# JuliaDSP/DSP.jl

Measured on NVIDIA H100. Metric: Gsamples/s filt+welch on 2^26 cplx-F32, higher is better.
Workload: dtype c64 (ComplexF32; f32 arithmetic)

## Files before the change

### __graft_entry__.py

```python
import os
import subprocess
import sys

ROOT = os.path.dirname(os.path.abspath(__file__))
PKG = os.path.join(ROOT, "dsp.jl_b200")


def build() -> None:
    jobs = str(min(8, os.cpu_count() or 2))
    subprocess.run(["make", "-C", os.path.join(PKG, "csrc"), "-j", jobs], check=True)
    host_dir = os.path.join(ROOT, "tests", "host")
    os.makedirs(os.path.join(ROOT, "build"), exist_ok=True)
    subprocess.run(["g++", "-std=c++17", "-O2", "-x", "c++", "-w", "-I/usr/local/cuda/include",
                    "-o", os.path.join(ROOT, "build", "fft_core_host_check"),
                    os.path.join(host_dir, "fft_core_host_check.cu")], check=True)
    for name in ("fir_tile_host_check", "fir_state_host_check"):
        subprocess.run(["g++", "-std=c++17", "-O2", "-march=native", "-x", "c++", "-w", "-I/usr/local/cuda/include",
                        "-o", os.path.join(ROOT, "build", name), os.path.join(host_dir, name + ".cu")], check=True)
    if ROOT not in sys.path:
        sys.path.insert(0, ROOT)
    import dspb200
    assert dspb200._lib.lib.dspb200_version() == 100


def smoke() -> None:
    if ROOT not in sys.path:
        sys.path.insert(0, ROOT)
    import numpy as np
    import dspb200
    from oracle import dspbase as od, periodograms as op, windows as ow

    if dspb200.device_count() < 1:
        raise RuntimeError("smoke() needs a CUDA device; dspb200 has no CPU fallback")
    rng = np.random.default_rng(7)
    x = (rng.standard_normal(1 << 16) + 1j * rng.standard_normal(1 << 16)).astype(np.complex64)
    v = (rng.standard_normal(513) + 1j * rng.standard_normal(513)).astype(np.complex64)
    y = dspb200.conv(x, v, algorithm="fft_overlapsave")
    ref = od.conv_exact(x, v)
    err = np.linalg.norm(y - ref) / np.linalg.norm(ref)
    assert y.dtype == np.complex64 and err < 1e-6, f"conv parity {err}"
    s = rng.standard_normal(1 << 18).astype(np.float32)
    p = dspb200.welch_pgram(s, 4096, 2048, window=dspb200.hanning)
    pref, _ = op.welch_pgram(s, 4096, 2048, window=ow.hanning, f64=True)
    err2 = np.linalg.norm(p.power - pref) / np.linalg.norm(pref)
    assert p.power.dtype == np.float32 and err2 < 1e-6, f"welch parity {err2}"
    print(f"smoke ok: conv relerr {err:.2e}, welch relerr {err2:.2e}, launches {dspb200.launch_count()}")


# ... 5 lines not shown
```

### dsp.jl_b200/csrc/fft_core.cuh

```cuda
#pragma once
#include "common.cuh"
#include <math.h>

#ifndef DSP_PROBE
#define DSP_PROBE 0
#endif

namespace dspb200 {

template <typename T> struct fft_pad { static constexpr int K = sizeof(T) == 4 ? 2 : 1; };
template <typename T> __host__ __device__ constexpr int fft_pad256(int n) {
    if (sizeof(T) == 4) return n == 512 ? 8 : (n == 1024 ? 4 : (n == 8192 ? 4 : 2));
    return n == 512 ? 4 : (n == 1024 ? 2 : (n == 8192 ? 2 : 1));
}
template <typename T> __host__ __device__ constexpr int fft_pad4096(int n) {
    if (sizeof(T) == 4) return n == 8192 ? 2 : (n == 16384 ? 4 : 0);
    return n == 8192 ? 1 : 0;
}
template <typename T, int N> __host__ __device__ __forceinline__ constexpr int padaddr(int p) {
    return p + fft_pad<T>::K * (p >> 4) + fft_pad256<T>(N) * (p >> 8) + fft_pad4096<T>(N) * (p >> 12);
}
template <typename T> __host__ __device__ constexpr int padded_len(int n) {
    return ((n - 1) + fft_pad<T>::K * ((n - 1) >> 4) + fft_pad256<T>(n) * ((n - 1) >> 8) + fft_pad4096<T>(n) * ((n - 1) >> 12) + 1 + 3) & ~3;
}
// ... 441 lines not shown
    } else {
        const int t = tp + Q * A;
        cx<T> w[RL / 2];
        if constexpr (N == 16384) {
            const cx<T> w1 = fft_tl_in_smem<T, N>() ? c.tl[t] : ldtw<T>(c.tl, t);
            w[1] = w1;
            w[0] = mkc<T>(fma_(w1.x, w1.x, -(w1.y * w1.y)), (w1.x + w1.x) * w1.y);
        } else {
#pragma unroll
            for (int i = 0; i < P::TLK; ++i) w[i] = fft_tl_in_smem<T, N>() ? c.tl[t * P::TLK + i] : ldtw<T>(c.tl, t * P::TLK + i);
        }
        fft_bfly<T, RL, false>(u, w);
    }
}

template <typename T, int N, int NT, class Ld0, class StLast>
__device__ __forceinline__ void fft_forward(const FftCtx<T>& c, int tid, Ld0 ld0, StLast stlast) {
    constexpr int Q = fft_plan_traits<N>::Q;
    constexpr int ITERS = (Q + NT - 1) / NT;
    fft_first_pass<T, N, NT, false>(c, tid, ld0);
    __syncthreads();
    fft_middle<T, N, NT>(c, tid);
#pragma unroll
    for (int it = 0; it < ITERS; ++it) {
        const int tp = tid + it * NT;
        if (Q % NT != 0 && tp >= Q) break;
        cx<T> v[16];
        fft_last_pass<T, N>(c, tp, v);
#pragma unroll
        for (int r = 0; r < 16; ++r) stlast(tp + r * Q, it, r, v[r]);
    }
}

template <typename T> inline void fft_fill_row(cx<T>* row, int R, long long num, long long den, int limit = 1 << 30) {
    const long double PI2 = 6.283185307179586476925286766559005768L;
    int qb = 0;
    for (int r = R; r > 1; r >>= 1) ++qb;
    int idx = 0;
    for (int k = 1; k <= qb; ++k) {
        const int cnt = k <= 2 ? 1 : (1 << (k - 2));
        for (int m = 0; m < cnt; ++m) {
            const long double a = -PI2 * ((long double)num * (long double)(R >> k) / (long double)den + (long double)m / (long double)(1 << k));
            if (idx < limit) row[idx] = mkc<T>((T)cosl(a), (T)sinl(a));
            ++idx;
        }
    }
}
template <typename T> inline void fft_fill_tables(cx<T>* t16, cx<T>* t256, long long n) {
    cx<T> row[8];
    const int nrow = fft_tw_row(n);
    const int keep6[6] = {0, 1, 2, 4, 5, 7};
    for (int t = 0; t < 16; ++t) {
        fft_fill_row<T>(row, 16, t, 256);
        for (int i = 0; i < nrow; ++i) t16[fft_tw_index<T>(i, t, 16)] = row[nrow == 8 ? i : keep6[i]];
    }
    for (int t = 0; t < 256; ++t) {
        fft_fill_row<T>(row, 16, t, 4096);
        for (int i = 0; i < nrow; ++i) t256[fft_tw_index<T>(i, t, 256)] = row[nrow == 8 ? i : keep6[i]];
    }
}
inline void fft_last_radix(long long n, int* rl, int* tlk) {
    int logn = 0;
    for (long long m = n; m > 1; m >>= 1) ++logn;
    const int ql = logn - 4;
    const int nmid = ql <= 4 ? 0 : (ql <= 8 ? 1 : 2);
    *rl = 1 << (ql - 4 * nmid);
    *tlk = *rl == 16 ? 0 : (n == 16384 ? 1 : *rl / 2);
}
inline long long fft_tl_len_rt(long long n) {
    int rl, tlk;
    fft_last_radix(n, &rl, &tlk);
    return (n / rl) * tlk;
}
template <typename T> inline void fft_fill_tl(cx<T>* tl, long long n) {
    int rl, tlk;
    fft_last_radix(n, &rl, &tlk);
    if (tlk == 0) return;
    const long double PI2 = 6.283185307179586476925286766559005768L;
    for (long long t = 0; t < n / rl; ++t) {
        if (n == 16384) {
            const long double a = -PI2 * (long double)t / (long double)n;
            tl[t] = mkc<T>((T)cosl(a), (T)sinl(a));
        } else {
            fft_fill_row<T>(tl + t * tlk, rl, t, n);
        }
    }
}

template <int N> struct fft_threads {
    static constexpr int NB16 = N / 16;
    static constexpr int value = NB16 < 64 ? 64 : (NB16 > 512 ? 512 : (NB16 > 256 ? 256 : NB16));
};
template <typename T, int N> struct fft_minblocks {
    static constexpr int value = sizeof(T) == 8 ? 1 : (fft_threads<N>::value >= 512 ? 1 : 512 / fft_threads<N>::value);
};

}
```

### dsp.jl_b200/csrc/overlap_save.cu

```cuda
#include "fft_core.cuh"
#include "async_copy.cuh"
#include "cufft_exec.cuh"
#include <math.h>
#include <stdlib.h>
#include <new>

namespace dspb200 {

struct OsPlanImpl {
    int dtype = 0;
    bool cplx = false, f64 = false;
    int64_t nv = 0, nfft = 0, L = 0;
    bool fused = false;
    int device = 0;
    void* d_tw = nullptr;
    void* d_t16 = nullptr;
    void* d_t256 = nullptr;
    int sm_count = 0;
    int fused_per_sm = 0;
    int fused_state_per_sm = 0;
    void* d_H = nullptr;
    cufftHandle fwd = 0, inv = 0;
    bool fft_ok = false;
    int64_t batch = 0, nbins = 0;
    DevBuf td, fd;
    HostPipe pipe;
};

template <typename T, bool CPLX> struct os_elt { using type = T; };
template <typename T> struct os_elt<T, true> { using type = cx<T>; };


template <typename T, int N, bool CPLX> struct os_threads {
    static constexpr bool f32 = sizeof(T) == 4;
    static constexpr int value = fft_threads<N>::value;
    static constexpr bool wide = f32 && ((N >= 512 && N <= 4096) || (N == 256 && !CPLX));
    static constexpr int minblocks = wide ? 1024 / value : fft_minblocks<T, N>::value;
    static constexpr bool staged = f32 && N == 16384;
};
constexpr int OS_STAGE_HEAD = 32768;
static_assert(OS_STAGE_HEAD % 16 == 0, "TMA copies move multiples of 16 bytes");
static_assert(OS_STAGE_HEAD < 16384 * 4, "the head region holds less than the shortest staged span (N + 1 floats)");
template <typename T, int N, bool CPLX> constexpr size_t os_smem_bytes() {
    return (size_t)fft_smem_elems<T, N>() * sizeof(cx<T>) + (os_threads<T, N, CPLX>::staged ? OS_STAGE_HEAD + 16 : 0);
}

template <typename T> __device__ __forceinline__ cx<T> ldg_cx(const cx<T>* __restrict__ p) {
    if constexpr (sizeof(T) == 4) {
        const float2 v = __ldg(reinterpret_cast<const float2*>(p));
        return mkc<T>(v.x, v.y);
    } else {
        const double2 v = __ldg(reinterpret_cast<const double2*>(p));
        return mkc<T>(v.x, v.y);
    }
}

template <typename E> struct OsUnit {
    const E* u;
    E* out;
    int jlo, jhi, jend, jzero;
    int nvm1, L;
};

template <typename E, bool STATE> struct OsState {};
template <typename E> struct OsState<E, true> {
    const E* si_in;
    E* si_out;
    int64_t nx;
};
template <typename E> struct OsUnitState {
    const E* si_in;
    E* si_out;
    int jsi, jnx;
};
struct OsNoState {};
template <typename E> __device__ __forceinline__ void os_put_state(const OsUnit<E>& g, const OsUnitState<E>& s, int j, E v) {
    if (j < s.jsi) v = v + s.si_in[j];
// ... 2 lines not shown
}

__device__ __forceinline__ int os_clamp(int64_t v) {
    return (int)(v < -(int64_t(1) << 30) ? -(int64_t(1) << 30) : (v > (int64_t(1) << 30) ? (int64_t(1) << 30) : v));
}
__device__ __forceinline__ int os_clamp_diff(int64_t a, int64_t b) {
    return a >= (int64_t(1) << 62) ? (1 << 30) : os_clamp(a - b);
}

template <typename T, bool CPLX, bool INTERIOR>
__device__ __forceinline__ cx<T> os_sample(const OsUnit<typename os_elt<T, CPLX>::type>& g, int j) {
#if DSP_PROBE & 2
    return mkc<T>(T(j), T(1));
#endif
    if constexpr (CPLX) {
        if constexpr (INTERIOR) return g.u[j];
        return (j >= g.jlo && j < g.jhi) ? g.u[j] : mkc<T>(T(0), T(0));
    } else {
        const int jb = j + g.L;
        if constexpr (INTERIOR) return mkc<T>(g.u[j], g.u[jb]);
        const T a = (j >= g.jlo && j < g.jhi) ? g.u[j] : T(0);
        const T b = (jb >= g.jlo && jb < g.jhi) ? g.u[jb] : T(0);
        return mkc<T>(a, b);
    }
}

struct OsStage {
    unsigned char* head;
    uint64_t* bar;
    uint32_t bytes;
    uint32_t parity;
};

template <typename T, int N, bool CPLX, int NT, bool INTERIOR, int ITERS, bool STATE, typename SG>
__device__ __forceinline__ void os_unit(const FftCtx<T>& ctx, int tid, const OsUnit<typename os_elt<T, CPLX>::type>& g,
                                        const cx<T>* __restrict__ H, OsStage& st, bool staged,
                                        const typename os_elt<T, CPLX>::type* __restrict__ next_u, const SG& state_geometry) {
    using E = typename os_elt<T, CPLX>::type;
    constexpr int Q = fft_plan_traits<N>::Q;
    constexpr bool STAGED = os_threads<T, N, CPLX>::staged;
    static_assert(ITERS == (Q + NT - 1) / NT, "register tile does not match the thread count");
    static_assert(!STAGED || (ITERS == 2 && Q % NT == 0), "TMA staging is laid out for two butterflies per thread");
    if (STAGED && INTERIOR && staged) {
        mbar_wait(st.bar, st.parity);
        st.parity ^= 1;
        const E* s = reinterpret_cast<const E*>(st.head);
        cx<T> v[ITERS][16];
#pragma unroll
        for (int it = 0; it < ITERS; ++it)
#pragma unroll
            for (int r = 0; r < 16; ++r) {
                const int j = tid + it * NT + r * Q;
                if constexpr (CPLX) v[it][r] = s[j];
                else v[it][r] = mkc<T>(s[j], s[j + g.L]);
            }
        fft_first_pass_regs<T, N, NT, true>(ctx, tid, v);
    } else {
        auto ld0 = [&](int j, int, int) -> cx<T> { return os_sample<T, CPLX, INTERIOR>(g, j); };
        fft_first_pass<T, N, NT, true>(ctx, tid, ld0);
    }
    __syncthreads();
    if (STAGED && next_u != nullptr && tid == 0) {
        fence_proxy_async_shared();
        mbar_expect_tx_noarrive(st.bar, OS_STAGE_HEAD);
        tma_load_1d(st.head, next_u, OS_STAGE_HEAD, st.bar);
    }
    fft_middle<T, N, NT>(ctx, tid);
    cx<T> v[ITERS][16];
#pragma unroll
    for (int it = 0; it < ITERS; ++it) {
        const int tp = tid + it * NT;
        if (Q % NT == 0 || tp < Q) {
            fft_last_pass<T, N, (ITERS == 1 && Q % NT == 0) ? NT : 0>(ctx, tp, v[it], tid);
#pragma unroll
#if DSP_PROBE & 4
            for (int r = 0; r < 16; ++r) v[it][r] = cswap(cmul(v[it][r], mkc<T>(T(0.5), T(r))));
#else
            for (int r = 0; r < 16; ++r) v[it][r] = cswap(cmul(v[it][r], ldg_cx<T>(H + tp + r * Q)));
#endif
            fft_bfly16_plain<T>(v[it]);
        }
    }
    __syncthreads();
#pragma unroll
    for (int it = 0; it < ITERS; ++it) {
        const int tp = tid + it * NT;
        if (Q % NT == 0 || tp < Q) fft_store_block<T, N>(ctx.sm, tp, v[it]);
    }
    __syncthreads();
    fft_middle<T, N, NT>(ctx, tid);
    constexpr int RL = fft_plan_traits<N>::RL, NBF = 16 / RL;
    using SGeom = std::conditional_t<STATE && !INTERIOR, OsUnitState<E>, OsNoState>;
    SGeom sg{};
    if constexpr (STATE && !INTERIOR) sg = state_geometry();
    auto put = [&](int j, cx<T> y) {
#if DSP_PROBE & 8
        if (y.x != T(123456.75)) return;
#endif
        if (j < g.nvm1) return;
        if constexpr (CPLX) {
            if constexpr (INTERIOR) g.out[j] = mkc<T>(y.y, y.x);
            else if constexpr (STATE) { if (j < g.jend) os_put_state(g, sg, j, mkc<T>(y.y, y.x)); }
            else if (j < g.jend) g.out[j] = (j < g.jzero) ? mkc<T>(y.y, y.x) : mkc<T>(T(0), T(0));
        } else {
            const int jb = j + g.L;
            if constexpr (INTERIOR) {
                g.out[j] = y.y;
                g.out[jb] = y.x;
            } else if constexpr (STATE) {
                if (j < g.jend) os_put_state(g, sg, j, y.y);
                if (jb < g.jend) os_put_state(g, sg, jb, y.x);
            } else {
                if (j < g.jend) g.out[j] = (j < g.jzero) ? y.y : T(0);
                if (jb < g.jend) g.out[jb] = (jb < g.jzero) ? y.x : T(0);
            }
        }
    };
    if constexpr (STAGED) {
        cx<T> w[ITERS][16];
#pragma unroll
        for (int it = 0; it < ITERS; ++it) fft_last_pass_load<T, N>(ctx, tid + it * NT, w[it]);
        if (next_u != nullptr) {
            __syncthreads();
            if (tid == 0) {
                fence_proxy_async_shared();
                mbar_expect_tx(st.bar, st.bytes - OS_STAGE_HEAD);
                tma_load_1d(ctx.sm, reinterpret_cast<const unsigned char*>(next_u) + OS_STAGE_HEAD, st.bytes - OS_STAGE_HEAD,
                            st.bar);
            }
        }
#pragma unroll
        for (int it = 0; it < ITERS; ++it) {
            const int tp = tid + it * NT;
            fft_last_pass_bfly<T, N>(ctx, tp, w[it]);
#pragma unroll
            for (int r = 0; r < 16; ++r) put(tp + r * Q, w[it][r]);
        }
    } else {
        auto chunk = [&](auto a_, int tp) {
            constexpr int A = decltype(a_)::value;
            cx<T> u[RL];
            fft_last_pass_chunk<T, N, A>(ctx, tp, u);
#pragma unroll
            for (int jj = 0; jj < RL; ++jj) put(tp + (A + NBF * jj) * Q, u[jj]);
        };
#pragma unroll
        for (int it = 0; it < ITERS; ++it) {
            const int tp = tid + it * NT;
            if (Q % NT != 0 && tp >= Q) break;
            chunk(std::integral_constant<int, 0>{}, tp);
            if constexpr (NBF >= 2) chunk(std::integral_constant<int, 1>{}, tp);
            if constexpr (NBF >= 4) { chunk(std::integral_constant<int, 2>{}, tp); chunk(std::integral_constant<int, 3>{}, tp); }
            if constexpr (NBF >= 8) {
                chunk(std::integral_constant<int, 4>{}, tp); chunk(std::integral_constant<int, 5>{}, tp);
                chunk(std::integral_constant<int, 6>{}, tp); chunk(std::integral_constant<int, 7>{}, tp);
            }
        }
    }
}

template <typename T, int N, bool CPLX, bool STATE>
__global__ void __launch_bounds__((os_threads<T, N, CPLX>::value), (os_threads<T, N, CPLX>::minblocks))
os_fused_kernel(const void* __restrict__ u_, int64_t u_begin, int64_t nu_local, int64_t u_col_stride,
                void* __restrict__ out_, int64_t out_begin, int64_t out_count, int64_t out_col_stride,
                int64_t zero_from, int nv, int64_t units_per_col, int64_t total_units, const cx<T>* __restrict__ gtl,
                const cx<T>* __restrict__ g16, const cx<T>* __restrict__ g256, const cx<T>* __restrict__ H,
                const OsState<typename os_elt<T, CPLX>::type, STATE> sa) {
    constexpr int NT = os_threads<T, N, CPLX>::value;
    constexpr int Q = fft_plan_traits<N>::Q;
    constexpr int ITERS = (Q + NT - 1) / NT;
    constexpr bool STAGED = os_threads<T, N, CPLX>::staged;
    extern __shared__ __align__(16) unsigned char smem_raw[];
    constexpr int HEAD = STAGED ? OS_STAGE_HEAD : 0;
    cx<T>* sm = reinterpret_cast<cx<T>*>(smem_raw + HEAD);
    using E = typename os_elt<T, CPLX>::type;
    const int tid = threadIdx.x;
    pdl_launch_dependents();
    const FftCtx<T> ctx = fft_make_ctx<T, N, NT>(sm, g16, g256, gtl, tid);
    OsStage st;
    st.head = smem_raw;
    st.bar = reinterpret_cast<uint64_t*>(smem_raw + HEAD + (size_t)fft_smem_elems<T, N>() * sizeof(cx<T>));
    st.parity = 0;
    if constexpr (STAGED) {
        if (tid == 0) {
            mbar_init(st.bar, 1);
            mbar_fence_init();
        }
    }
    pdl_wait();
    __syncthreads();
    const int L = N - nv + 1;
    const int span = CPLX ? N : N + L;
    st.bytes = (uint32_t)((span * sizeof(E) + 15) & ~(size_t)15);

    const bool onecol = units_per_col >= total_units;
    auto geometry = [&](int64_t gu, OsUnit<E>& g) -> bool {
        const int64_t col = onecol ? 0 : gu / units_per_col;
        const int64_t unit = gu - col * units_per_col;
        const int64_t q = CPLX ? unit : 2 * unit;
        const int64_t s0 = out_begin + q * L - (nv - 1);
        const int64_t i0 = s0 - u_begin;
        g.u = reinterpret_cast<const E*>(u_) + col * u_col_stride + i0;
        g.out = reinterpret_cast<E*>(out_) + col * out_col_stride + (s0 - out_begin);
        g.jlo = os_clamp(-i0);
        g.jhi = os_clamp(nu_local - i0);
        g.jend = os_clamp(out_begin + out_count - s0);
        g.jzero = os_clamp_diff(zero_from, s0);
        g.nvm1 = nv - 1;
        g.L = L;
        return g.jlo <= 0 && g.jhi >= span && g.jend >= span && g.jzero >= span;
    };
    auto state_geometry = [&](int64_t gu) {
        OsUnitState<E> s{};
        if constexpr (STATE) {
// ... 14 lines not shown
            int64_t lo = out_begin + qn * L - (nv - 1) - u_begin;
            int64_t hi = lo + span;
            if (lo < 0) lo = 0;
            if (hi > nu_local) hi = nu_local;
            const uintptr_t a0 = ((uintptr_t)(reinterpret_cast<const E*>(u_) + coln * u_col_stride + lo) + 15) & ~(uintptr_t)15;
            const uintptr_t a1 = (uintptr_t)(reinterpret_cast<const E*>(u_) + coln * u_col_stride + hi) & ~(uintptr_t)15;
            if (hi > lo && a1 > a0) tma_prefetch_l2(reinterpret_cast<const void*>(a0), (uint32_t)(a1 - a0));
        }
    };
    auto stage_src = [&](int64_t gn) -> const E* {
        if (!STAGED || gn >= total_units || (DSP_PROBE & 2)) return nullptr;
        OsUnit<E> gl;
        if (!geometry(gn, gl)) return nullptr;
        if ((int64_t)gl.jhi * (int64_t)sizeof(E) < (int64_t)st.bytes || ((uintptr_t)gl.u & 15) != 0) return nullptr;
        return gl.u;
    };
    bool staged = false;
    if constexpr (STAGED) {
        const E* src = stage_src(blockIdx.x);
        staged = src != nullptr;
        if (staged && tid == 0) {
            mbar_expect_tx(st.bar, st.bytes);
            tma_load_1d(st.head, src, OS_STAGE_HEAD, st.bar);
            tma_load_1d(ctx.sm, reinterpret_cast<const unsigned char*>(src) + OS_STAGE_HEAD, st.bytes - OS_STAGE_HEAD, st.bar);
        }
    }

    for (int64_t gu = blockIdx.x; gu < total_units; gu += gridDim.x) {
        l2_prefetch(gu + (int64_t)gridDim.x);
        OsUnit<E> g;
        const bool interior = geometry(gu, g);
        const E* next_u = stage_src(gu + gridDim.x);
        auto sgeom = [&]() { return state_geometry(gu); };
        if (interior) os_unit<T, N, CPLX, NT, true, ITERS, STATE>(ctx, tid, g, H, st, staged, next_u, sgeom);
        else os_unit<T, N, CPLX, NT, false, ITERS, STATE>(ctx, tid, g, H, st, staged, next_u, sgeom);
        staged = next_u != nullptr;
    }
}

template <typename T, int N, bool CPLX>
__global__ void __launch_bounds__(fft_threads<N>::value, fft_minblocks<T, N>::value)
os_filter_kernel(const void* __restrict__ v_, int nv, const cx<T>* __restrict__ gtl, const cx<T>* __restrict__ g16,
                 const cx<T>* __restrict__ g256, cx<T>* __restrict__ H) {
    constexpr int NT = fft_threads<N>::value;
    extern __shared__ __align__(16) unsigned char smem_raw[];
    cx<T>* sm = reinterpret_cast<cx<T>*>(smem_raw);
    using E = typename os_elt<T, CPLX>::type;
    const E* v = reinterpret_cast<const E*>(v_);
    const FftCtx<T> ctx = fft_make_ctx<T, N, NT>(sm, g16, g256, gtl, threadIdx.x);
    __syncthreads();
    const T scale = T(1) / T(N);
    auto ld0 = [&](int j, int, int) -> cx<T> {
        if (j >= nv) return mkc<T>(T(0), T(0));
        if constexpr (CPLX) return v[j]; else return mkc<T>(v[j], T(0));
    };
    auto stl = [&](int k, int, int, cx<T> x) { H[k] = cscale(x, scale); };
    fft_forward<T, N, NT>(ctx, threadIdx.x, ld0, stl);
}

template <typename T, bool CPLX>
__global__ void os_gather_kernel(const void* __restrict__ u_, int64_t u_begin, int64_t nu_local, int64_t m_first,
                                 int64_t L, int64_t nv, int64_t nfft, int64_t nblk, void* __restrict__ td_) {
    using E = typename os_elt<T, CPLX>::type;
    const E* u = reinterpret_cast<const E*>(u_);
    E* td = reinterpret_cast<E*>(td_);
    const int64_t total = nblk * nfft;
    for (int64_t i = (int64_t)blockIdx.x * blockDim.x + threadIdx.x; i < total; i += (int64_t)gridDim.x * blockDim.x) {
        const int64_t b = i / nfft, j = i - b * nfft;
// ... 174 lines not shown
    void* si_out;
    int64_t nx;
};
constexpr int OS_STATE_MIN_NFFT = 1024;
template <typename E, bool STATE> static OsState<E, STATE> os_state_arg(const OsStateArgs& s, int64_t off) {
    OsState<E, STATE> r{};
    if constexpr (STATE)
        r = {s.si_in ? reinterpret_cast<const E*>(s.si_in) + off : nullptr, s.si_out ? reinterpret_cast<E*>(s.si_out) + off : nullptr, s.nx};
    return r;
}

template <typename T, int N, bool CPLX, bool STATE>
static int launch_os_fused(OsPlanImpl* p, const OsRange& a, const OsStateArgs& s, cudaStream_t st) {
    using E = typename os_elt<T, CPLX>::type;
    constexpr int NT = os_threads<T, N, CPLX>::value;
    const size_t smem = os_smem_bytes<T, N, CPLX>();
    auto kern = os_fused_kernel<T, N, CPLX, STATE>;
    const OsState<E, STATE> sa = os_state_arg<E, STATE>(s, 0);
    const int64_t nblk = cdiv(a.out_count, p->L);
    const int64_t upc = CPLX ? nblk : (nblk + 1) / 2;
    const int64_t units = upc * a.ncols;
    if (units < 1) return DSPB200_OK;
    int& per_sm = STATE ? p->fused_state_per_sm : p->fused_per_sm;
    if (per_sm < 1) {
        DSP_TRY(set_smem(kern, smem));
        int per = 1;
        DSP_CUDA(cudaOccupancyMaxActiveBlocksPerMultiprocessor(&per, kern, NT, smem));
        per_sm = per < 1 ? 1 : per;
    }
    const int64_t cap = (int64_t)p->sm_count * per_sm;
    const int64_t blocks = units < cap ? units : cap;
    DSP_CUDA(launch_pdl(kern, (unsigned)blocks, NT, smem, st, a.u, a.u_begin, a.nu_local, a.u_col_stride, a.out, a.out_begin,
                        a.out_count, a.out_col_stride, a.zero_from, (int)p->nv, upc, units,
                        reinterpret_cast<const cx<T>*>(p->d_tw), reinterpret_cast<const cx<T>*>(p->d_t16),
                        reinterpret_cast<const cx<T>*>(p->d_t256), reinterpret_cast<const cx<T>*>(p->d_H), sa));
    DSP_LAUNCH_OK();
    return DSPB200_OK;
}

template <typename T, bool STATE> static int os_fused_dispatch(OsPlanImpl* p, const OsRange& a, const OsStateArgs& s, cudaStream_t st) {
    switch (p->nfft) {
#define X(NN)                                                                                                       \
    case NN:                                                                                                        \
        if constexpr ((sizeof(T) == 8 && NN > 8192) || (STATE && NN < OS_STATE_MIN_NFFT)) break;                    \
        else return p->cplx ? launch_os_fused<T, NN, true, STATE>(p, a, s, st) : launch_os_fused<T, NN, false, STATE>(p, a, s, st);
        DSP_OS_SIZES(X)
#undef X
    }
    set_error("no fused %soverlap-save kernel for nfft=%lld", STATE ? "stateful " : "", (long long)p->nfft);
    return DSPB200_EUNSUPPORTED;
}

template <typename T, int N, bool CPLX>
static int launch_os_filter(OsPlanImpl* p, const void* d_v) {
    constexpr int NT = fft_threads<N>::value;
    const size_t smem = (size_t)fft_smem_elems<T, N>() * sizeof(cx<T>);
    auto kern = os_filter_kernel<T, N, CPLX>;
    DSP_TRY(set_smem(kern, smem));
    kern<<<1, NT, smem, 0>>>(d_v, (int)p->nv, reinterpret_cast<const cx<T>*>(p->d_tw), reinterpret_cast<const cx<T>*>(p->d_t16),
                             reinterpret_cast<const cx<T>*>(p->d_t256), reinterpret_cast<cx<T>*>(p->d_H));
    DSP_LAUNCH_OK();
    DSP_CUDA(cudaStreamSynchronize(0));
    return DSPB200_OK;
}

template <typename T> static int os_filter_dispatch(OsPlanImpl* p, const void* d_v) {
    switch (p->nfft) {
#define X(NN)                                                                                   \
// ... 202 lines not shown
    });
}

extern "C" {

int dspb200_os_plan_create(dspb200_os_plan** plan, int dtype, const void* v_host, int64_t nv, int64_t nfft) {
    DSP_RANGE("dspb200_os_plan_create");
    DSP_REQUIRE(plan != nullptr, "plan is NULL");
    *plan = nullptr;
    DSP_REQUIRE(dtype_valid(dtype), "invalid dtype %d", dtype);
    DSP_REQUIRE(v_host != nullptr && nv >= 1, "filter must be non-empty");
    DSP_REQUIRE(nfft == 0 || nfft >= nv, "nfft (%lld) must be >= nv (%lld)", (long long)nfft, (long long)nv);
    DSP_REQUIRE(nfft < (int64_t(1) << 30), "nfft too large");
    dspb200_os_plan* h = new (std::nothrow) dspb200_os_plan();
    DSP_REQUIRE(h != nullptr, "out of host memory");
    OsPlanImpl* p = &h->impl;
    p->dtype = dtype; p->cplx = dtype_is_cplx(dtype); p->f64 = dtype_is_f64(dtype);
    p->nv = nv;
    p->nfft = nfft ? nfft : auto_nfft(nv, p->f64);
    p->L = p->nfft - nv + 1;
    p->fused = os_fused_ok(p->nfft, nv, p->f64);
    const size_t esz = dtype_size(dtype), csz = p->f64 ? 16 : 8;
    int rc = DSPB200_OK;
    void* d_v = nullptr;
    do {
        cudaError_t e = cudaGetDevice(&p->device);
        if (e != cudaSuccess) { rc = cuda_fail(e, "cudaGetDevice", __FILE__, __LINE__); break; }
        rc = upload(&d_v, v_host, (size_t)nv * esz);
        if (rc != DSPB200_OK) break;
        if (p->fused) {
            p->sm_count = device_sm_count();
            rc = upload_fft_tables(p->nfft, p->f64, &p->d_tw, &p->d_t16, &p->d_t256);
            if (rc != DSPB200_OK) break;
            e = cudaMalloc(&p->d_H, (size_t)p->nfft * csz);
            if (e != cudaSuccess) { rc = cuda_fail(e, "cudaMalloc(H)", __FILE__, __LINE__); break; }
            rc = p->f64 ? os_filter_dispatch<double>(p, d_v) : os_filter_dispatch<float>(p, d_v);
        } else {
            p->nbins = p->cplx ? p->nfft : p->nfft / 2 + 1;
            int64_t b = (int64_t(1) << 22) / p->nfft;
            if (b < 1) b = 1;
            if (b > 4096) b = 4096;
            p->batch = b;
            rc = fft_plan_1d(&p->fwd, p->cplx, p->f64, CUFFT_FORWARD, p->nfft, b);
            if (rc == DSPB200_OK) rc = fft_plan_1d(&p->inv, p->cplx, p->f64, CUFFT_INVERSE, p->nfft, b);
            if (rc != DSPB200_OK) break;
            p->fft_ok = true;
            rc = p->td.reserve((size_t)(b * p->nfft) * esz);
            if (rc == DSPB200_OK) rc = p->fd.reserve((size_t)(b * p->nbins) * csz);
            if (rc != DSPB200_OK) break;
            e = cudaMalloc(&p->d_H, (size_t)p->nbins * csz);
            if (e != cudaSuccess) { rc = cuda_fail(e, "cudaMalloc(H)", __FILE__, __LINE__); break; }
            e = cudaMemset(p->td.p, 0, (size_t)(b * p->nfft) * esz);
            if (e != cudaSuccess) { rc = cuda_fail(e, "cudaMemset", __FILE__, __LINE__); break; }
            const int threads = 256;
            if (p->f64) {
                if (p->cplx) pad_copy_kernel<double, true><<<grid_for(p->nfft, threads), threads>>>(d_v, nv, p->td.p, p->nfft, 1.0 / (double)p->nfft);
                else pad_copy_kernel<double, false><<<grid_for(p->nfft, threads), threads>>>(d_v, nv, p->td.p, p->nfft, 1.0 / (double)p->nfft);
            } else {
                if (p->cplx) pad_copy_kernel<float, true><<<grid_for(p->nfft, threads), threads>>>(d_v, nv, p->td.p, p->nfft, 1.0f / (float)p->nfft);
                else pad_copy_kernel<float, false><<<grid_for(p->nfft, threads), threads>>>(d_v, nv, p->td.p, p->nfft, 1.0f / (float)p->nfft);
            }
            count_launch(1);
            rc = fft_exec(p->fwd, p->cplx, p->f64, CUFFT_FORWARD, p->td.p, p->fd.p, 0);
            if (rc != DSPB200_OK) break;
            e = cudaMemcpy(p->d_H, p->fd.p, (size_t)p->nbins * csz, cudaMemcpyDeviceToDevice);
            if (e == cudaSuccess) e = cudaDeviceSynchronize();
// ... 89 lines not shown
            const int64_t m0 = c * chunk_out, cnt = nout - m0 < chunk_out ? nout - m0 : chunk_out;
            int64_t i_lo = m0 - (p->nv - 1); if (i_lo < 0) i_lo = 0;
            int64_t i_hi = m0 + cnt; if (i_hi > nu) i_hi = nu;
            const int64_t ni = i_hi > i_lo ? i_hi - i_lo : 0;
            auto run = [=, &hp](const void* in, void* o) {
                return os_run(p, OsRange{in, i_lo, ni, 0, o, m0, cnt, 0, nfull, 1}, hp.s_exec);
            };
            return {(const char*)u + (size_t)i_lo * esz, (size_t)ni * esz, run, nullptr, (char*)out + (size_t)m0 * esz, (size_t)cnt * esz};
        };
        return run_chunked(hp, cdiv(nout, chunk_out), (size_t)(chunk_out + p->nv - 1) * esz, (size_t)chunk_out * esz, chunk, nullptr);
    }
    return run_staged(hp.s_exec, {{u, (size_t)(nu * ncols) * esz, &hp.in[0]}}, {{out, (size_t)(nout * ncols) * esz, &hp.out[0]}},
                      [&] { return dspb200_os_exec_dev(plan, hp.in[0].p, nu, ncols, hp.out[0].p, nout, hp.s_exec); });
}

int dspb200_os_exec_state(dspb200_os_plan* plan, const void* x, int64_t nx, int64_t ncols, const void* si_in, void* si_out,
                          void* out) {
    DSP_RANGE("dspb200_os_exec_state");
    DSP_REQUIRE(plan != nullptr, "plan is NULL");
    OsPlanImpl* p = &plan->impl;
    HostPipe& hp = p->pipe;
    return exec_state_host(p, hp.s_exec, x, nx, ncols, si_in, si_out, out, p->nv - 1, dtype_size(p->dtype), hp.in[0], hp.out[0],
                           hp.in[1], hp.out[1], [&](const void* d_x, const void* d_si_in, void* d_si_out, void* d_out) {
                               return dspb200_os_exec_state_dev(plan, d_x, nx, ncols, d_si_in, d_si_out, d_out, hp.s_exec);
                           });
}

int dspb200_os_plan_destroy(dspb200_os_plan* plan) {
    if (!plan) return DSPB200_OK;
    OsPlanImpl* p = &plan->impl;
    if (p->d_tw) cudaFree(p->d_tw);
    if (p->d_t16) cudaFree(p->d_t16);
    if (p->d_t256) cudaFree(p->d_t256);
    if (p->d_H) cudaFree(p->d_H);
    if (p->fft_ok) { cufftDestroy(p->fwd); cufftDestroy(p->inv); }
    p->td.release(); p->fd.release();
    p->pipe.release();
    delete plan;
    return DSPB200_OK;
}

int dspb200_conv_fft_exec(int dtype, const void* u, int64_t nu, const void* v, int64_t nv, int64_t nfft, void* out) {
    DSP_RANGE("dspb200_conv_fft_exec");
    DSP_TRY(conv_nd_check(dtype, ND_FFT, 1, &nu, u, &nv, v, &nfft, out));
    return conv_nd_run_host(dtype, ND_FFT, 1, &nu, u, &nv, v, &nfft, out);
}

int dspb200_conv_nd_exec(int dtype, int rank, const int64_t* usize, const void* u, const int64_t* vsize, const void* v,
                         const int64_t* nffts, void* out) {
    DSP_RANGE("dspb200_conv_nd_exec");
    const int mode = nffts ? ND_FFT : ND_DIRECT;
    DSP_TRY(conv_nd_check(dtype, mode, rank, usize, u, vsize, v, nffts, out));
    return conv_nd_run_host(dtype, mode, rank, usize, u, vsize, v, nffts, out);
}
int dspb200_conv_nd_exec_dev(int dtype, int rank, const int64_t* usize, const void* d_u, const int64_t* vsize, const void* d_v,
                             const int64_t* nffts, void* d_out, void* stream) {
    DSP_RANGE("dspb200_conv_nd_exec_dev");
    const int mode = nffts ? ND_FFT : ND_DIRECT;
    DSP_TRY(conv_nd_check(dtype, mode, rank, usize, d_u, vsize, d_v, nffts, d_out));
    return conv_nd_run_dev(dtype, mode, rank, usize, d_u, vsize, d_v, nffts, d_out, reinterpret_cast<cudaStream_t>(stream));
}

int dspb200_conv_nd_os_exec(int dtype, int rank, const int64_t* usize, const void* u, const int64_t* vsize, const void* v,
                            const int64_t* nffts, void* out) {
    DSP_RANGE("dspb200_conv_nd_os_exec");
    DSP_TRY(conv_nd_check(dtype, ND_OS, rank, usize, u, vsize, v, nffts, out));
// ... 59 lines not shown
```

Baseline: 73.04.

## Use radix-32 three-pass FFT for staged 16384-point overlap-save kernel

Adds a dedicated radix-32 x 32 x 16 FFT decomposition for N=16384 f32 in the TMA-staged overlap-save path, with its own padded shared-memory layout and compact twiddle table. The last-pass twiddles are derived from two loaded values by squaring and constant multiplies. The goal is fewer shared-memory passes and barriers per unit than the generic radix-16 plan. In exchange it raises register pressure (32-element register tiles) and adds a new code path and table upload.

```diff
diff --git a/__graft_entry__.py b/__graft_entry__.py
--- a/__graft_entry__.py
+++ b/__graft_entry__.py
@@ -11,9 +11,9 @@
     subprocess.run(["make", "-C", os.path.join(PKG, "csrc"), "-j", jobs], check=True)
     host_dir = os.path.join(ROOT, "tests", "host")
     os.makedirs(os.path.join(ROOT, "build"), exist_ok=True)
-    subprocess.run(["g++", "-std=c++17", "-O2", "-x", "c++", "-w", "-I/usr/local/cuda/include",
-                    "-o", os.path.join(ROOT, "build", "fft_core_host_check"),
-                    os.path.join(host_dir, "fft_core_host_check.cu")], check=True)
+    for name in ("fft_core_host_check", "fft_r32_host_check"):
+        subprocess.run(["g++", "-std=c++17", "-O2", "-x", "c++", "-w", "-I/usr/local/cuda/include",
+                        "-o", os.path.join(ROOT, "build", name), os.path.join(host_dir, name + ".cu")], check=True)
     for name in ("fir_tile_host_check", "fir_state_host_check"):
         subprocess.run(["g++", "-std=c++17", "-O2", "-march=native", "-x", "c++", "-w", "-I/usr/local/cuda/include",
                         "-o", os.path.join(ROOT, "build", name), os.path.join(host_dir, name + ".cu")], check=True)
diff --git a/dsp.jl_b200/csrc/fft_core.cuh b/dsp.jl_b200/csrc/fft_core.cuh
--- a/dsp.jl_b200/csrc/fft_core.cuh
+++ b/dsp.jl_b200/csrc/fft_core.cuh
@@ -497,6 +497,78 @@
     }
 }
 
+struct fft_r32 {
+    static constexpr int N = 16384;
+    static constexpr int NT = 512;
+    static constexpr int Q = N / 32;
+    static constexpr int QL = N / 16;
+    static constexpr int T32_LEN = 32 * 16;
+    static constexpr int TL_LEN = 2 * QL;
+    static constexpr int TABLE_LEN = T32_LEN + TL_LEN;
+    static constexpr int C10 = 2;
+    static constexpr int PADDED_LEN = ((N - 1) + C10 * ((N - 1) >> 10) + 1 + 3) & ~3;
+    static constexpr int SMEM_ELEMS = PADDED_LEN + TABLE_LEN;
+};
+__host__ __device__ __forceinline__ constexpr int fft_r32_padaddr(int p) { return p + fft_r32::C10 * (p >> 10); }
+__host__ __device__ __forceinline__ constexpr int fft_r32_block_of(int c) { return 32 * (c & 15) + (c >> 4); }
+
+template <typename T> struct FftR32Ctx {
+    cx<T>* sm;
+    const cx<T>* t32;
+    const cx<T>* tl;
+};
+template <typename T>
+__device__ __forceinline__ FftR32Ctx<T> fft_r32_make_ctx(cx<T>* data, cx<T>* tabs, const cx<T>* __restrict__ g, int tid) {
+    for (int i = tid; i < fft_r32::TABLE_LEN; i += fft_r32::NT) tabs[i] = g[i];
+    return FftR32Ctx<T>{data, tabs, tabs + fft_r32::T32_LEN};
+}
+
+template <typename T> __host__ __device__ __forceinline__ void fft_r32_first_bfly(cx<T> (&v)[32]) { fft_bfly<T, 32, true>(v, nullptr); }
+template <typename T> __host__ __device__ __forceinline__ void fft_r32_store_block(cx<T>* sm, int c, const cx<T> (&v)[32]) {
+    cx<T>* p = sm + fft_r32_padaddr(32 * fft_r32_block_of(c));
+#pragma unroll
+    for (int r = 0; r < 32; r += 2) sts2<T>(p + r, v[r], v[r + 1]);
+}
+
+template <typename T, bool GATE = false> __host__ __device__ __forceinline__ void fft_r32_middle(const FftR32Ctx<T>& c, int tid) {
+    const int t = tid & 31;
+    cx<T>* p = c.sm + fft_r32_padaddr((tid >> 5) * 1024 + t);
+    cx<T> v[32], w[16];
+    if constexpr (GATE) fft_gate_wait<fft_r32::NT>(tid);
+#pragma unroll
+    for (int i = 0; i < 16; i += 2) lds2<T>(c.t32 + fft_tw_index<T>(i, t, 32), w[i], w[i + 1]);
+#pragma unroll
+    for (int r = 0; r < 32; ++r) v[r] = p[32 * r];
+    if constexpr (GATE) fft_gate_open<fft_r32::NT>(tid);
+    fft_bfly<T, 32, false>(v, w);
+#pragma unroll
+    for (int r = 0; r < 32; ++r) p[32 * r] = v[r];
+}
+
+template <typename T> __host__ __device__ __forceinline__ void fft_r32_last_load(const FftR32Ctx<T>& c, int t, cx<T> (&v)[16]) {
+    const cx<T>* p = c.sm + fft_r32_padaddr(t);
+#pragma unroll
+    for (int s = 0; s < 16; ++s) v[s] = p[fft_r32_padaddr(s * 1024)];
+}
+template <typename T> __host__ __device__ __forceinline__ cx<T> fft_sq(cx<T> a) {
+    return mkc<T>(fma_(a.x, a.x, -(a.y * a.y)), (a.x + a.x) * a.y);
+}
+template <typename T> __host__ __device__ __forceinline__ cx<T> fft_mul_const(cx<T> a, T cr, T ci) {
+    return mkc<T>(fma_(a.x, cr, -(a.y * ci)), fma_(a.x, ci, a.y * cr));
+}
+template <typename T> __host__ __device__ __forceinline__ void fft_r32_last_bfly(const FftR32Ctx<T>& c, int t, cx<T> (&v)[16]) {
+    const T c16 = fft_const<T>::C8, s16 = fft_const<T>::S8;
+    cx<T> w[8];
+    lds2<T>(c.tl + 2 * t, w[1], w[4]);
+    w[2] = fft_sq(w[4]);
+    w[0] = fft_sq(w[1]);
+    w[3] = mul_w8<T>(w[2]);
+    w[5] = fft_mul_const<T>(w[4], c16, -s16);
+    w[6] = mul_w8<T>(w[4]);
+    w[7] = fft_mul_const<T>(w[4], s16, -c16);
+    fft_bfly<T, 16, false>(v, w);
+}
+
 template <typename T> inline void fft_fill_row(cx<T>* row, int R, long long num, long long den, int limit = 1 << 30) {
     const long double PI2 = 6.283185307179586476925286766559005768L;
     int qb = 0;
@@ -552,6 +624,20 @@
     }
 }
 
+template <typename T> inline void fft_r32_fill_tables(cx<T>* tab) {
+    cx<T> row[16];
+    for (int t = 0; t < 32; ++t) {
+        fft_fill_row<T>(row, 32, t, 1024);
+        for (int i = 0; i < 16; ++i) tab[fft_tw_index<T>(i, t, 32)] = row[i];
+    }
+    const long double PI2 = 6.283185307179586476925286766559005768L;
+    for (int t = 0; t < fft_r32::QL; ++t) {
+        const long double a = -PI2 * (long double)t / (long double)fft_r32::N;
+        tab[fft_r32::T32_LEN + 2 * t] = mkc<T>((T)cosl(4 * a), (T)sinl(4 * a));
+        tab[fft_r32::T32_LEN + 2 * t + 1] = mkc<T>((T)cosl(a), (T)sinl(a));
+    }
+}
+
 template <int N> struct fft_threads {
     static constexpr int NB16 = N / 16;
     static constexpr int value = NB16 < 64 ? 64 : (NB16 > 512 ? 512 : (NB16 > 256 ? 256 : NB16));
diff --git a/dsp.jl_b200/csrc/overlap_save.cu b/dsp.jl_b200/csrc/overlap_save.cu
--- a/dsp.jl_b200/csrc/overlap_save.cu
+++ b/dsp.jl_b200/csrc/overlap_save.cu
@@ -4,6 +4,7 @@
 #include <math.h>
 #include <stdlib.h>
 #include <new>
+#include <vector>
 
 namespace dspb200 {
 
@@ -16,6 +17,7 @@
     void* d_tw = nullptr;
     void* d_t16 = nullptr;
     void* d_t256 = nullptr;
+    void* d_r32 = nullptr;
     int sm_count = 0;
     int fused_per_sm = 0;
     int fused_state_per_sm = 0;
@@ -41,8 +43,11 @@
 constexpr int OS_STAGE_HEAD = 32768;
 static_assert(OS_STAGE_HEAD % 16 == 0, "TMA copies move multiples of 16 bytes");
 static_assert(OS_STAGE_HEAD < 16384 * 4, "the head region holds less than the shortest staged span (N + 1 floats)");
+template <typename T, int N, bool CPLX> __host__ __device__ constexpr int os_fft_elems() {
+    return os_threads<T, N, CPLX>::staged ? fft_r32::SMEM_ELEMS : fft_smem_elems<T, N>();
+}
 template <typename T, int N, bool CPLX> constexpr size_t os_smem_bytes() {
-    return (size_t)fft_smem_elems<T, N>() * sizeof(cx<T>) + (os_threads<T, N, CPLX>::staged ? OS_STAGE_HEAD + 16 : 0);
+    return (size_t)os_fft_elems<T, N, CPLX>() * sizeof(cx<T>) + (os_threads<T, N, CPLX>::staged ? OS_STAGE_HEAD + 16 : 0);
 }
 
 template <typename T> __device__ __forceinline__ cx<T> ldg_cx(const cx<T>* __restrict__ p) {
@@ -111,39 +116,43 @@
     uint32_t parity;
 };
 
+template <typename T, bool CPLX, bool INTERIOR, bool STATE, typename SGeom>
+__device__ __forceinline__ void os_put(const OsUnit<typename os_elt<T, CPLX>::type>& g, const SGeom& sg, int j, cx<T> y) {
+#if DSP_PROBE & 8
+    if (y.x != T(123456.75)) return;
+#endif
+    if (j < g.nvm1) return;
+    if constexpr (CPLX) {
+        if constexpr (INTERIOR) g.out[j] = mkc<T>(y.y, y.x);
+        else if constexpr (STATE) { if (j < g.jend) os_put_state(g, sg, j, mkc<T>(y.y, y.x)); }
+        else if (j < g.jend) g.out[j] = (j < g.jzero) ? mkc<T>(y.y, y.x) : mkc<T>(T(0), T(0));
+    } else {
+        const int jb = j + g.L;
+        if constexpr (INTERIOR) {
+            g.out[j] = y.y;
+            g.out[jb] = y.x;
+        } else if constexpr (STATE) {
+            if (j < g.jend) os_put_state(g, sg, j, y.y);
+            if (jb < g.jend) os_put_state(g, sg, jb, y.x);
+        } else {
+            if (j < g.jend) g.out[j] = (j < g.jzero) ? y.y : T(0);
+            if (jb < g.jend) g.out[jb] = (jb < g.jzero) ? y.x : T(0);
+        }
+    }
+}
+template <typename E, bool STATE, bool INTERIOR> using os_sgeom_t = std::conditional_t<STATE && !INTERIOR, OsUnitState<E>, OsNoState>;
+
 template <typename T, int N, bool CPLX, int NT, bool INTERIOR, int ITERS, bool STATE, typename SG>
 __device__ __forceinline__ void os_unit(const FftCtx<T>& ctx, int tid, const OsUnit<typename os_elt<T, CPLX>::type>& g,
-                                        const cx<T>* __restrict__ H, OsStage& st, bool staged,
-                                        const typename os_elt<T, CPLX>::type* __restrict__ next_u, const SG& state_geometry) {
+                                        const cx<T>* __restrict__ H, const SG& state_geometry) {
     using E = typename os_elt<T, CPLX>::type;
     constexpr int Q = fft_plan_traits<N>::Q;
-    constexpr bool STAGED = os_threads<T, N, CPLX>::staged;
     static_assert(ITERS == (Q + NT - 1) / NT, "register tile does not match the thread count");
-    static_assert(!STAGED || (ITERS == 2 && Q % NT == 0), "TMA staging is laid out for two butterflies per thread");
-    if (STAGED && INTERIOR && staged) {
-        mbar_wait(st.bar, st.parity);
-        st.parity ^= 1;
-        const E* s = reinterpret_cast<const E*>(st.head);
-        cx<T> v[ITERS][16];
-#pragma unroll
-        for (int it = 0; it < ITERS; ++it)
-#pragma unroll
-            for (int r = 0; r < 16; ++r) {
-                const int j = tid + it * NT + r * Q;
-                if constexpr (CPLX) v[it][r] = s[j];
-                else v[it][r] = mkc<T>(s[j], s[j + g.L]);
-            }
-        fft_first_pass_regs<T, N, NT, true>(ctx, tid, v);
-    } else {
+    {
         auto ld0 = [&](int j, int, int) -> cx<T> { return os_sample<T, CPLX, INTERIOR>(g, j); };
         fft_first_pass<T, N, NT, true>(ctx, tid, ld0);
     }
     __syncthreads();
-    if (STAGED && next_u != nullptr && tid == 0) {
-        fence_proxy_async_shared();
-        mbar_expect_tx_noarrive(st.bar, OS_STAGE_HEAD);
-        tma_load_1d(st.head, next_u, OS_STAGE_HEAD, st.bar);
-    }
     fft_middle<T, N, NT>(ctx, tid);
     cx<T> v[ITERS][16];
 #pragma unroll
@@ -169,72 +178,104 @@
     __syncthreads();
     fft_middle<T, N, NT>(ctx, tid);
     constexpr int RL = fft_plan_traits<N>::RL, NBF = 16 / RL;
-    using SGeom = std::conditional_t<STATE && !INTERIOR, OsUnitState<E>, OsNoState>;
-    SGeom sg{};
+    os_sgeom_t<E, STATE, INTERIOR> sg{};
     if constexpr (STATE && !INTERIOR) sg = state_geometry();
-    auto put = [&](int j, cx<T> y) {
-#if DSP_PROBE & 8
-        if (y.x != T(123456.75)) return;
+    auto chunk = [&](auto a_, int tp) {
+        constexpr int A = decltype(a_)::value;
+        cx<T> u[RL];
+        fft_last_pass_chunk<T, N, A>(ctx, tp, u);
+#pragma unroll
+        for (int jj = 0; jj < RL; ++jj) os_put<T, CPLX, INTERIOR, STATE>(g, sg, tp + (A + NBF * jj) * Q, u[jj]);
+    };
+#pragma unroll
+    for (int it = 0; it < ITERS; ++it) {
+        const int tp = tid + it * NT;
+        if (Q % NT != 0 && tp >= Q) break;
+        chunk(std::integral_constant<int, 0>{}, tp);
+        if constexpr (NBF >= 2) chunk(std::integral_constant<int, 1>{}, tp);
+        if constexpr (NBF >= 4) { chunk(std::integral_constant<int, 2>{}, tp); chunk(std::integral_constant<int, 3>{}, tp); }
+        if constexpr (NBF >= 8) {
+            chunk(std::integral_constant<int, 4>{}, tp); chunk(std::integral_constant<int, 5>{}, tp);
+            chunk(std::integral_constant<int, 6>{}, tp); chunk(std::integral_constant<int, 7>{}, tp);
+        }
+    }
+}
+
+template <typename T, bool CPLX, bool INTERIOR, bool STATE, typename SG>
+__device__ __forceinline__ void os_unit_r32(const FftR32Ctx<T>& ctx, int tid, const OsUnit<typename os_elt<T, CPLX>::type>& g,
+                                            const cx<T>* __restrict__ H, OsStage& st, bool staged,
+                                            const typename os_elt<T, CPLX>::type* __restrict__ next_u, const SG& state_geometry) {
+    using E = typename os_elt<T, CPLX>::type;
+    constexpr int NT = fft_r32::NT, Q = fft_r32::Q;
+    cx<T> v[32];
+    if (INTERIOR && staged) {
+        mbar_wait(st.bar, st.parity);
+        st.parity ^= 1;
+        const E* s = reinterpret_cast<const E*>(st.head);
+#pragma unroll
+        for (int m = 0; m < 32; ++m) {
+            const int j = tid + m * Q;
+            if constexpr (CPLX) v[m] = s[j];
+            else v[m] = mkc<T>(s[j], s[j + g.L]);
+        }
+    } else {
+#pragma unroll
+        for (int m = 0; m < 32; ++m) v[m] = os_sample<T, CPLX, INTERIOR>(g, tid + m * Q);
+    }
+    fft_r32_first_bfly<T>(v);
+    __syncthreads();
+    fft_r32_store_block<T>(ctx.sm, tid, v);
+    __syncthreads();
+    if (next_u != nullptr && tid == 0) {
+        fence_proxy_async_shared();
+        mbar_expect_tx_noarrive(st.bar, OS_STAGE_HEAD);
+        tma_load_1d(st.head, next_u, OS_STAGE_HEAD, st.bar);
+    }
+#if !(DSP_PROBE & 16)
+    fft_r32_middle<T, true>(ctx, tid);
 #endif
-        if (j < g.nvm1) return;
-        if constexpr (CPLX) {
-            if constexpr (INTERIOR) g.out[j] = mkc<T>(y.y, y.x);
-            else if constexpr (STATE) { if (j < g.jend) os_put_state(g, sg, j, mkc<T>(y.y, y.x)); }
-            else if (j < g.jend) g.out[j] = (j < g.jzero) ? mkc<T>(y.y, y.x) : mkc<T>(T(0), T(0));
-        } else {
-            const int jb = j + g.L;
-            if constexpr (INTERIOR) {
-                g.out[j] = y.y;
-                g.out[jb] = y.x;
-            } else if constexpr (STATE) {
-                if (j < g.jend) os_put_state(g, sg, j, y.y);
-                if (jb < g.jend) os_put_state(g, sg, jb, y.x);
-            } else {
-                if (j < g.jend) g.out[j] = (j < g.jzero) ? y.y : T(0);
-                if (jb < g.jend) g.out[jb] = (jb < g.jzero) ? y.x : T(0);
-            }
-        }
-    };
-    if constexpr (STAGED) {
-        cx<T> w[ITERS][16];
+    __syncthreads();
+    {
+        cx<T> u[2][16];
 #pragma unroll
-        for (int it = 0; it < ITERS; ++it) fft_last_pass_load<T, N>(ctx, tid + it * NT, w[it]);
-        if (next_u != nullptr) {
-            __syncthreads();
-            if (tid == 0) {
-                fence_proxy_async_shared();
-                mbar_expect_tx(st.bar, st.bytes - OS_STAGE_HEAD);
-                tma_load_1d(ctx.sm, reinterpret_cast<const unsigned char*>(next_u) + OS_STAGE_HEAD, st.bytes - OS_STAGE_HEAD,
-                            st.bar);
-            }
+        for (int it = 0; it < 2; ++it) {
+            fft_r32_last_load<T>(ctx, tid + it * NT, u[it]);
+            fft_r32_last_bfly<T>(ctx, tid + it * NT, u[it]);
         }
 #pragma unroll
-        for (int it = 0; it < ITERS; ++it) {
-            const int tp = tid + it * NT;
-            fft_last_pass_bfly<T, N>(ctx, tp, w[it]);
+#if DSP_PROBE & 4
+        for (int m = 0; m < 32; ++m) v[m] = cswap(cmul(u[m & 1][m >> 1], mkc<T>(T(0.5), T(m))));
+#else
+        for (int m = 0; m < 32; ++m) v[m] = cswap(cmul(u[m & 1][m >> 1], ldg_cx<T>(H + tid + m * Q)));
+#endif
+    }
+    fft_r32_first_bfly<T>(v);
+    __syncthreads();
+    fft_r32_store_block<T>(ctx.sm, tid, v);
+    __syncthreads();
+#if !(DSP_PROBE & 16)
+    fft_r32_middle<T, true>(ctx, tid);
+#endif
+    __syncthreads();
+    os_sgeom_t<E, STATE, INTERIOR> sg{};
+    if constexpr (STATE && !INTERIOR) sg = state_geometry();
+    cx<T> w[2][16];
 #pragma unroll
-            for (int r = 0; r < 16; ++r) put(tp + r * Q, w[it][r]);
-        }
-    } else {
-        auto chunk = [&](auto a_, int tp) {
-            constexpr int A = decltype(a_)::value;
-            cx<T> u[RL];
-            fft_last_pass_chunk<T, N, A>(ctx, tp, u);
+    for (int it = 0; it < 2; ++it) fft_r32_last_load<T>(ctx, tid + it * NT, w[it]);
+    if (next_u != nullptr) {
+        __syncthreads();
+        if (tid == 0) {
+            fence_proxy_async_shared();
+            mbar_expect_tx(st.bar, st.bytes - OS_STAGE_HEAD);
+            tma_load_1d(ctx.sm, reinterpret_cast<const unsigned char*>(next_u) + OS_STAGE_HEAD, st.bytes - OS_STAGE_HEAD, st.bar);
+        }
+    }
 #pragma unroll
-            for (int jj = 0; jj < RL; ++jj) put(tp + (A + NBF * jj) * Q, u[jj]);
-        };
+    for (int it = 0; it < 2; ++it) {
+        const int t = tid + it * NT;
+        fft_r32_last_bfly<T>(ctx, t, w[it]);
 #pragma unroll
-        for (int it = 0; it < ITERS; ++it) {
-            const int tp = tid + it * NT;
-            if (Q % NT != 0 && tp >= Q) break;
-            chunk(std::integral_constant<int, 0>{}, tp);
-            if constexpr (NBF >= 2) chunk(std::integral_constant<int, 1>{}, tp);
-            if constexpr (NBF >= 4) { chunk(std::integral_constant<int, 2>{}, tp); chunk(std::integral_constant<int, 3>{}, tp); }
-            if constexpr (NBF >= 8) {
-                chunk(std::integral_constant<int, 4>{}, tp); chunk(std::integral_constant<int, 5>{}, tp);
-                chunk(std::integral_constant<int, 6>{}, tp); chunk(std::integral_constant<int, 7>{}, tp);
-            }
-        }
+        for (int s = 0; s < 16; ++s) os_put<T, CPLX, INTERIOR, STATE>(g, sg, t + s * fft_r32::QL, w[it][s]);
     }
 }
 
@@ -255,10 +296,14 @@
     using E = typename os_elt<T, CPLX>::type;
     const int tid = threadIdx.x;
     pdl_launch_dependents();
-    const FftCtx<T> ctx = fft_make_ctx<T, N, NT>(sm, g16, g256, gtl, tid);
+    auto make_ctx = [&]() {
+        if constexpr (STAGED) return fft_r32_make_ctx<T>(sm, sm + fft_r32::PADDED_LEN, gtl, tid);
+        else return fft_make_ctx<T, N, NT>(sm, g16, g256, gtl, tid);
+    };
+    const auto ctx = make_ctx();
     OsStage st;
     st.head = smem_raw;
-    st.bar = reinterpret_cast<uint64_t*>(smem_raw + HEAD + (size_t)fft_smem_elems<T, N>() * sizeof(cx<T>));
+    st.bar = reinterpret_cast<uint64_t*>(smem_raw + HEAD + (size_t)os_fft_elems<T, N, CPLX>() * sizeof(cx<T>));
     st.parity = 0;
     if constexpr (STAGED) {
         if (tid == 0) {
@@ -339,8 +384,13 @@
         const bool interior = geometry(gu, g);
         const E* next_u = stage_src(gu + gridDim.x);
         auto sgeom = [&]() { return state_geometry(gu); };
-        if (interior) os_unit<T, N, CPLX, NT, true, ITERS, STATE>(ctx, tid, g, H, st, staged, next_u, sgeom);
-        else os_unit<T, N, CPLX, NT, false, ITERS, STATE>(ctx, tid, g, H, st, staged, next_u, sgeom);
+        if constexpr (STAGED) {
+            if (interior) os_unit_r32<T, CPLX, true, STATE>(ctx, tid, g, H, st, staged, next_u, sgeom);
+            else os_unit_r32<T, CPLX, false, STATE>(ctx, tid, g, H, st, staged, next_u, sgeom);
+        } else {
+            if (interior) os_unit<T, N, CPLX, NT, true, ITERS, STATE>(ctx, tid, g, H, sgeom);
+            else os_unit<T, N, CPLX, NT, false, ITERS, STATE>(ctx, tid, g, H, sgeom);
+        }
         staged = next_u != nullptr;
     }
 }
@@ -581,8 +631,9 @@
     const int64_t blocks = units < cap ? units : cap;
     DSP_CUDA(launch_pdl(kern, (unsigned)blocks, NT, smem, st, a.u, a.u_begin, a.nu_local, a.u_col_stride, a.out, a.out_begin,
                         a.out_count, a.out_col_stride, a.zero_from, (int)p->nv, upc, units,
-                        reinterpret_cast<const cx<T>*>(p->d_tw), reinterpret_cast<const cx<T>*>(p->d_t16),
-                        reinterpret_cast<const cx<T>*>(p->d_t256), reinterpret_cast<const cx<T>*>(p->d_H), sa));
+                        reinterpret_cast<const cx<T>*>(os_threads<T, N, CPLX>::staged ? p->d_r32 : p->d_tw),
+                        reinterpret_cast<const cx<T>*>(p->d_t16), reinterpret_cast<const cx<T>*>(p->d_t256),
+                        reinterpret_cast<const cx<T>*>(p->d_H), sa));
     DSP_LAUNCH_OK();
     return DSPB200_OK;
 }
@@ -851,6 +902,12 @@
             p->sm_count = device_sm_count();
             rc = upload_fft_tables(p->nfft, p->f64, &p->d_tw, &p->d_t16, &p->d_t256);
             if (rc != DSPB200_OK) break;
+            if (!p->f64 && p->nfft == fft_r32::N) {
+                std::vector<cx<float>> tab(fft_r32::TABLE_LEN);
+                fft_r32_fill_tables<float>(tab.data());
+                rc = upload(&p->d_r32, tab.data(), tab.size() * sizeof(cx<float>));
+                if (rc != DSPB200_OK) break;
+            }
             e = cudaMalloc(&p->d_H, (size_t)p->nfft * csz);
             if (e != cudaSuccess) { rc = cuda_fail(e, "cudaMalloc(H)", __FILE__, __LINE__); break; }
             rc = p->f64 ? os_filter_dispatch<double>(p, d_v) : os_filter_dispatch<float>(p, d_v);
@@ -1006,6 +1063,7 @@
     if (p->d_tw) cudaFree(p->d_tw);
     if (p->d_t16) cudaFree(p->d_t16);
     if (p->d_t256) cudaFree(p->d_t256);
+    if (p->d_r32) cudaFree(p->d_r32);
     if (p->d_H) cudaFree(p->d_H);
     if (p->fft_ok) { cufftDestroy(p->fwd); cufftDestroy(p->inv); }
     p->td.release(); p->fd.release();
```

After: 76.25 (median of 6 runs). 4.4% higher.
